# facebookresearch/momentum

Hardware: NVIDIA H100
Metric: GN iterations/sec (batched 72-joint IK) (higher is better)
Workload: dtype f32

## Files before the change

momentum_b200/csrc/ik_capi.cu:

```cuda
#include "../../include/momentum_b200.h"

#include <cuda_runtime.h>
#include <nvtx3/nvToolsExt.h>

#include <algorithm>
#include <cfloat>
#include <cmath>
#include <cstdio>
#include <cstdlib>
#include <cstring>
#include <memory>
#include <string>
#include <vector>

#include "ik_chol_sched.h"
#include "ik_fused.cuh"
#include "ik_jtj_tc.cuh"
#include "ik_kernels.cuh"
#include "ik_plan.h"
#include "ik_solve_path.h"

using namespace mb2;

namespace {
// ... 139 lines not shown
  DeviceBuffer<ContribDesc> dContribs;
  DeviceBuffer<float> dLimitData;
  DeviceBuffer<int32_t> dEnabledList, dIdentity, dDeviceCols;
  DeviceBuffer<float> dTargets, dWeights, dJ, dTheta, dState, dH, dTargetStage;
  DeviceBuffer<double> dErrors;
  DeviceBuffer<double> dJacobi;
  std::unique_ptr<DeviceSchedule> sched;
  SweepLaunch lastSweep[2]{};
  FunctionTables tables() const;
};

struct PhaseEvent {
  cudaEvent_t start, stop;
  int phase;
};

struct mb2_solver {
  mb2_solver_function* fn{nullptr};
  mb2_gauss_newton_options opt{};
  DeviceBuffer<float> dH, dDelta, dThetaOrig, dTheta0, dScale, dGradDotDelta, dThetaStage, dGrad, dTiles, dRadius, dRSaved;
  DeviceBuffer<double> dLastErrors, dTrialErrors, dHistory;
  DeviceBuffer<int32_t> dActive, dIterations, dStatus, dSearching, dActiveCount, dWorkCounter, dQrChunks;
  DeviceBuffer<unsigned long long> dPhaseCycles;
  DeviceBuffer<float> dPark;
  DeviceBuffer<uint32_t> dParkSlots;
  SolvePath path;
  cudaEvent_t fusedStart{nullptr}, fusedStop{nullptr};
  double fusedMs{0};
  int* hActiveCount{nullptr};
  char* hResults{nullptr};
  size_t hResultsBytes{0};
  bool resultsStaged{false};
  uint64_t totalIterations{0}, kernelLaunches{0};
  bool profiling{false};
  bool inKernelProfile{false};
  std::vector<PhaseEvent> events;
  double phaseMs[4]{0, 0, 0, 0};
  uint64_t phaseLaunches[4]{0, 0, 0, 0};
  size_t historyStride{0};
  ~mb2_solver() {
    if (hActiveCount) cudaFreeHost(hActiveCount);
    if (hResults) cudaFreeHost(hResults);
    if (fusedStart) cudaEventDestroy(fusedStart);
    if (fusedStop) cudaEventDestroy(fusedStop);
    for (auto& e : events) { cudaEventDestroy(e.start); cudaEventDestroy(e.stop); }
  }
};

// ... 1397 lines not shown
  c.tilesStride = tilesStride;
  TrQrArgs t{};
  t.q.c = c;
  t.q.jacobian = f->dJ.p;
  t.q.numCols = f->plan.numCols;
  t.q.ldJ = f->ldJ;
  t.q.chunkStart = s->dQrChunks.p;
  t.q.numChunks = int32_t(P.qrChunkStarts.size()) - 1;
  t.T = f->tables();
  t.targets = f->dTargets.p;
  t.cweights = f->dWeights.p;
  t.radius = s->dRadius.p;
  t.rSaved = s->dRSaved.p;
  t.maxRadius = 10.f;
  t.maxChunkRows = P.qrWidestChunk;
  GramCholArgs gc{};
  gc.g = g;
  gc.c = c;
  gc.c.tilesIn = nullptr;
  gc.phaseCycles = s->inKernelProfile ? s->dPhaseCycles.p : nullptr;
  GramCholGlobalTables gt{};
  if (P.kind == kSolveGramCholesky) {
    const DeviceSchedule& ds = *f->sched;
    gc.parkTiles = ds.gc.parkTiles;
    if (gc.parkTiles > 0) {
      const int slots = gramCholeskyParkSlots(gc, ds.dev, ds.gcParams != nullptr);
      if (slots < 1) {
        s->path = SolvePath{};
        return fail(MB2_ERR_CUDA, "Gram + Cholesky fusion: no resident CTA");
      }
      if (s->dParkSlots.n < size_t(slots / 32)) {
        MB2_CUDA(s->dParkSlots.resize(size_t(slots / 32)));
        MB2_CUDA(cudaMemsetAsync(s->dParkSlots.p, 0, s->dParkSlots.n * sizeof(uint32_t), st));
      }
      MB2_CUDA(s->dPark.resize(size_t(slots) * size_t(gc.parkTiles) * 256));
      gc.park = s->dPark.p;
      gc.parkSlots = s->dParkSlots.p;
      gc.parkSlotWords = int32_t(slots / 32);
    }
    gt.L = ds.gc.L;
    gt.tab = ds.gcTab.p;
  }
  CholArgs& step = qr ? t.q.c : (P.kind == kSolveGramCholesky ? gc.c : c);
  SweepArgs trial = sweepArgs(f, theta, s->dSearching.p);
  trial.errors = s->dTrialErrors.p;
  LineSearchArgs la{};
  la.batch = B; la.ns = ns; la.numParams = n; la.ldTheta = n;
  la.errors = f->dErrors.p;
  la.trialErrors = s->dTrialErrors.p;
  la.gradDotDelta = s->dGradDotDelta.p;
  la.scale = s->dScale.p;
  la.searching = s->dSearching.p;
  la.subsetVariant = o.subset_line_search;
  la.active = s->dActive.p;
  BookkeepingArgs ba{};
  ba.batch = B;
  ba.errors = f->dErrors.p; ba.lastErrors = s->dLastErrors.p; ba.active = s->dActive.p; ba.iterations = s->dIterations.p;
  ba.status = s->dStatus.p; ba.history = history;
  ba.theta = theta; ba.ldTheta = n; ba.numParams = n;
  ba.minIterations = minIt; ba.maxIterations = maxIt; ba.threshold = o.threshold; ba.activeCount = s->dActiveCount.p;

  s->kernelLaunches = 0;
// ... 235 lines not shown
```

momentum_b200/csrc/ik_chol_sched.cpp:

```cpp
#include "ik_chol_sched.h"

#include "ik_chol_sched.cuh"

#include <algorithm>
#include <cstdio>
#include <cstdlib>
#include <map>
#include <set>
#include <tuple>

namespace mb2 {

namespace {

struct BitRows {
  int n, words;
  std::vector<uint64_t> b;
  BitRows(int n_) : n(n_), words((n_ + 63) / 64), b(size_t(n_) * ((n_ + 63) / 64), 0) {}
  uint64_t* row(int i) { return b.data() + size_t(i) * words; }
  const uint64_t* row(int i) const { return b.data() + size_t(i) * words; }
  void set(int i, int j) { row(i)[j >> 6] |= 1ull << (j & 63); }
  void clear(int i, int j) { row(i)[j >> 6] &= ~(1ull << (j & 63)); }
  bool test(int i, int j) const { return (row(i)[j >> 6] >> (j & 63)) & 1ull; }
  int count(int i) const {
// ... 342 lines not shown
      if (stripsOfQuad[q] != stripsOfQuad[q0] || stripId[{q, K}] != stripId[{q0, K}] + (q - q0) * stripsOfQuad[q0]) return "Gram plan: row quads of one unit are not laid out uniformly";
  }
  out.colStripStart.assign(T + 1, 0);
  for (int K = 0; K < T; ++K) {
    out.colStripStart[K + 1] = out.colStripStart[K] + int(ofCol[K].size());
    out.colStrip.insert(out.colStrip.end(), ofCol[K].begin(), ofCol[K].end());
  }
  return "";
}

void makeGramBlob(const GramPlan& g, const CholSchedule& s, std::vector<int32_t>& blob, int32_t offsets[8]) {
  blob.clear();
  int k = 0;
  auto add = [&](const std::vector<int32_t>& v) { offsets[k++] = int32_t(blob.size()); blob.insert(blob.end(), v.begin(), v.end()); while (blob.size() % 4) blob.push_back(0); };
  add(g.tileOrder); add(g.tileQuadStart); add(g.quad); add(std::vector<int32_t>()); add(g.colStripStart); add(g.colStrip);
  std::vector<int32_t> stripRow(g.numStrips), info(s.numTiles);
  for (int i = 0; i < g.numStrips; ++i) stripRow[i] = g.stripCoord[2 * i];
  auto validOf = [&](int K) { int v = 0; while (v < kCholTile && s.perm[16 * K + v] >= 0) ++v; return v; };
  for (int t = 0; t < s.numTiles; ++t) info[t] = validOf(s.tileRow[t]) | (validOf(s.tileCol[t]) << 8) | ((s.tileRow[t] == s.tileCol[t] ? 1 : 0) << 16);
  add(stripRow); add(info);
  if (blob.empty()) blob.push_back(0);
}

std::string makeGramCholTables(const GramPlan& g, const CholSchedule& s, GramCholTables& out) {
  out = GramCholTables();
  std::vector<uint16_t>& t = out.tab;
  bool fits = true;
  auto put = [&](int64_t v) { fits = fits && v >= 0 && v <= 0xFFFF; t.push_back(uint16_t(v)); };
  auto section = [&]() { while (t.size() % 4) t.push_back(0); return int32_t(t.size()); };
  auto validOf = [&](int K) { int v = 0; while (v < kCholTile && s.perm[16 * K + v] >= 0) ++v; return v; };
  out.L.gram = section();
  for (int32_t tile : g.tileOrder) {
    if (tile < 0) { put(0xFFFF); put(0); put(0); put(0); continue; }
    fits = fits && tile < 0xFFFF;
    put(tile);
    put(validOf(s.tileRow[tile]) | (validOf(s.tileCol[tile]) << 8) | ((s.tileRow[tile] == s.tileCol[tile] ? 1 : 0) << 15));
    put(g.tileQuadStart[tile]); put(g.tileQuadStart[tile + 1]);
  }
  out.L.quad = section();
  for (int32_t v : g.quad) put(v);
  out.L.col = section();
  for (int32_t v : g.colStripStart) put(v);
  out.L.colEnt = section();
  for (int32_t sidx : g.colStrip) { put(int64_t(sidx) * 64); put(g.stripCoord[2 * sidx]); }
  out.L.level = section();
  for (int L = 0; L <= s.numLevels; ++L) { put(s.levelColStart[L]); put(s.levelPanelStart[L]); put(s.levelOrderStart8[L]); put(s.levelVTaskStart[L]); }
  out.L.diag = section();
  for (int32_t K : s.levelCols) { put(K); put(s.diagTile[K]); put(s.colPanelStart[K]); put(s.colPanelStart[K + 1]); }
  out.L.panel = section();
  for (size_t pi = 0; pi < s.panelTile.size(); ++pi) { put(s.panelTile[pi]); put(s.panelDiag[pi]); }
  out.L.order = section();
  for (int32_t ti : s.taskOrder8) {
    if (ti < 0) { put(0xFFFF); put(0); put(0); put(0); continue; }
    fits = fits && s.taskDst[ti] < 0xFFFF;
    put(s.taskDst[ti]); put(s.taskPairStart[ti]); put(s.taskPairStart[ti + 1]); put(0);
  }
  out.L.pair = section();
  for (size_t p = 0; p < s.pairA.size(); ++p) { put(s.pairA[p]); put(s.pairB[p]); }
  out.L.vtask = section();
  for (size_t vi = 0; vi < s.vtaskRow.size(); ++vi) { put(s.vtaskRow[vi]); put(s.vtaskSrcStart[vi]); put(s.vtaskSrcStart[vi + 1]); put(0); }
  out.L.vsrc = section();
  for (size_t p = 0; p < s.vsrcTile.size(); ++p) { put(s.vsrcTile[p]); put(s.vsrcCol[p]); }
  out.L.colPanel = section();
  for (size_t p = 0; p < s.colPanelTile.size(); ++p) { put(s.colPanelTile[p]); put(s.colPanelRow[p]); }
  section();
  const int64_t onStrips = (int64_t(g.stride) + 64 + 255) / 256;
  out.parkTiles = int32_t(std::min<int64_t>(s.numTiles, onStrips));
  return fits ? "" : "Gram + Cholesky tables: an entry does not fit in 16 bits";
}

void layoutDeviceColumns(CholSchedule& s, std::vector<int32_t>& deviceColumnOrder) {
  deviceColumnOrder.clear();
  s.nParams = s.n;
  for (int K = 0; K < s.numTileCols; ++K) {
    while (deviceColumnOrder.size() % 4 != 0) deviceColumnOrder.push_back(-1);
    for (int j = 0; j < kCholTile; ++j) {
      int16_t& p = s.perm[16 * K + j];
      if (p < 0) continue;
      const int dev = int(deviceColumnOrder.size());
      deviceColumnOrder.push_back(p);
      p = int16_t(dev);
    }
  }
  s.n = int32_t(deviceColumnOrder.size());
  s.pos.assign(s.n, int16_t(-1));
  for (int slot = 0; slot < s.nPad; ++slot) if (s.perm[slot] >= 0) s.pos[s.perm[slot]] = int16_t(slot);
  s.order.assign(deviceColumnOrder.begin(), deviceColumnOrder.end());
}

}

// ... 43 lines not shown
```

momentum_b200/csrc/ik_chol_sched.h:

```cpp
#pragma once

#include <cstdint>
#include <string>
#include <vector>

namespace mb2 {

constexpr int kCholTile = 16;

struct CholSchedule {
  int32_t n{0}, nPad{0}, numTileCols{0}, numTiles{0}, numLevels{0};
  int32_t nParams{0};
  std::vector<int16_t> perm;
  std::vector<int16_t> pos;
  std::vector<int16_t> tileIdTable;
  std::vector<int16_t> tileRow, tileCol;
  std::vector<int32_t> diagTile;
  std::vector<int32_t> levelColStart, levelCols;
  std::vector<int32_t> levelPanelStart, panelTile, panelDiag, panelRow;
  std::vector<int32_t> levelTaskStart, taskDst, taskPairStart, pairA, pairB;
  std::vector<int32_t> levelOrderStart8, taskOrder8, levelOrderStart16, taskOrder16;
  std::vector<int32_t> levelVTaskStart, vtaskRow, vtaskSrcStart, vsrcTile, vsrcCol;
  std::vector<int32_t> colPanelStart, colPanelTile, colPanelRow;
  std::vector<int> order;
// ... 12 lines not shown
  std::vector<int32_t> stripCoord;
  std::vector<int32_t> tileOrder;
  std::vector<int32_t> tilePairStart;
  std::vector<int32_t> pairA, pairB;
  std::vector<int32_t> tileQuadStart;
  std::vector<int32_t> quad;
  std::vector<int32_t> colStripStart;
  std::vector<int32_t> colStrip;
  std::vector<uint32_t> cellStripOff;
  std::vector<uint16_t> cellQuadStride;
  int32_t residOff{0};
  int32_t stride{0};
  int64_t macs{0};
};
std::string buildGramPlan(const CholSchedule& s, const std::vector<int32_t>& cellRow0, const std::vector<int32_t>& cellRows, const std::vector<int32_t>& cellCol,
                          int numRows, GramPlan& out);

void makeGramBlob(const GramPlan& g, const CholSchedule& s, std::vector<int32_t>& blob, int32_t offsets[8]);

struct CholSchedDev;
void makeScheduleBlob(const CholSchedule& s, std::vector<int32_t>& blob, CholSchedDev& dev);

struct GramCholLayout {
  int32_t gram, quad, col, colEnt, level, diag, panel, order, pair, vtask, vsrc, colPanel;
};
struct GramCholTables {
  GramCholLayout L{};
  std::vector<uint16_t> tab;
  int32_t parkTiles{0};
};
std::string makeGramCholTables(const GramPlan& g, const CholSchedule& s, GramCholTables& out);

}
```

momentum_b200/csrc/ik_kernels.cu:

```cuda
#include "ik_kernels.cuh"

#include <algorithm>
#include <cstdio>
#include <type_traits>

#include "ik_chol.cuh"
#include "ik_chol_sched.h"
#include "ik_jtj_tc.cuh"
#include "ik_ptx.cuh"
#include "ik_device.cuh"
#include "ik_jacobi.cuh"

namespace mb2 {

__device__ __forceinline__ double warpSum(double v) {
  for (int o = 16; o > 0; o >>= 1) v += __shfl_xor_sync(0xffffffffu, v, o);
  return v;
}

size_t sweepSmemPerInstance(const FunctionTables& T, int warpsPerInstance) {
  const size_t nPad = (T.numParams + 3) & ~3;
  const size_t jp = warpsPerInstance > 1 ? size_t((T.numJoints * kParametersPerJoint + 1) & ~1) : 0;
  return sizeof(float) * (nPad + jp + size_t((T.numJoints * kJointStateStride + 1) & ~1) + size_t((T.recStride + 1) & ~1) + 4 + 2 * size_t(warpsPerInstance));
}
// ... 1874 lines not shown
  const bool prof = (a.profile & 1) != 0;
  cudaError_t e;
  if (wide) e = prof ? cudaFuncSetAttribute(choleskyScheduledKernel<512, true>, cudaFuncAttributeMaxDynamicSharedMemorySize, int(smem))
                     : cudaFuncSetAttribute(choleskyScheduledKernel<512, false>, cudaFuncAttributeMaxDynamicSharedMemorySize, int(smem));
  else e = prof ? cudaFuncSetAttribute(choleskyScheduledKernel<256, true>, cudaFuncAttributeMaxDynamicSharedMemorySize, int(smem))
                : cudaFuncSetAttribute(choleskyScheduledKernel<256, false>, cudaFuncAttributeMaxDynamicSharedMemorySize, int(smem));
  if (e != cudaSuccess) return e;
  if (a.tilesIn == nullptr && (a.g == nullptr || a.ldG != cholGradientLd(a.ns))) return cudaErrorInvalidValue;
  if ((a.ldH & 3) != 0 || (a.hStride & 3) != 0 || (a.tilesStride & 3) != 0) return cudaErrorInvalidValue;
  CUtensorMap hmap;
  const bool fromGram = a.tilesIn != nullptr;
  const uint64_t dims[3] = {uint64_t(fromGram ? 256 : a.ldH), uint64_t(fromGram ? sched.numTiles : a.ns + 1), uint64_t(a.batch)};
  const uint64_t strides[2] = {uint64_t(fromGram ? 256 : a.ldH) * sizeof(float), uint64_t(fromGram ? a.tilesStride : a.hStride) * sizeof(float)};
  const uint32_t box[3] = {16u, 16u, 1u};
  e = makeTensorMap3d(&hmap, fromGram ? a.tilesIn : a.H, dims, strides, box, 64);
  if (e != cudaSuccess) return e;
  if (wide && prof) choleskyScheduledKernel<512, true><<<a.batch, 512, smem, stream>>>(hmap, a, sched);
  else if (wide) choleskyScheduledKernel<512, false><<<a.batch, 512, smem, stream>>>(hmap, a, sched);
  else if (prof) choleskyScheduledKernel<256, true><<<a.batch, 256, smem, stream>>>(hmap, a, sched);
  else choleskyScheduledKernel<256, false><<<a.batch, 256, smem, stream>>>(hmap, a, sched);
  return cudaGetLastError();
}

__device__ int acquireParkSlot(uint32_t* words, int numWords, int start) {
  for (int w = start % numWords;; w = (w + 1 == numWords) ? 0 : w + 1) {
    uint32_t freeBits = ~__ldcg(words + w);
    while (freeBits != 0u) {
      const int bit = __ffs(freeBits) - 1;
      if ((atomicOr(words + w, 1u << bit) & (1u << bit)) == 0u) return 32 * w + bit;
      freeBits &= freeBits - 1u;
    }
  }
}

template <bool kProfile, class Tables>
__global__ void __launch_bounds__(kGramThreads, 4) gramCholeskyKernel(const GramCholArgs a, const CholSchedDev S, const __grid_constant__ Tables P) {
  extern __shared__ __align__(16) float gcSmem[];
  const GramArgs& g = a.g;
  const CholArgs& c = a.c;
  const int b = blockIdx.x;
  if (c.active[b] == 0) return;
  const int n = c.ns, tid = threadIdx.x;
  const int warp = tid >> 5, lane = tid & 31, hw = tid >> 4, hl = tid & 15;
  constexpr int kWarps = kGramThreads / 32;
  float* U = gcSmem + (((128u - (smemAddr(gcSmem) & 127u)) & 127u) >> 2);
  const size_t tileFloats = size_t(S.numTiles) * 256, sweepFloats = g.stripStride + 64;
  const size_t uni = ((tileFloats > sweepFloats ? tileFloats : sweepFloats) + 3) & ~size_t(3);
  float* strips = U;
  float* resid = U + g.residOff;
  float* tiles = U;
  float* y = U + uni;
  float* gsub = y + S.nPad;
  int* flags = reinterpret_cast<int*>(gsub + ((n + 3) & ~3));
  unsigned long long* bar = reinterpret_cast<unsigned long long*>(flags + 4);
  const uint16_t* tab = P.tab;
  const GramCholLayout& L = P.L;
  long long pc[8] = {0, 0, 0, 0, 0, 0, 0, 0}, pt = 0;
  if constexpr (kProfile) pt = clock64();
#define MB2_GC(k) if constexpr (kProfile) { const long long now = clock64(); pc[k] += now - pt; pt = now; }
  const uint32_t barAddr = smemAddr(bar);
  const uint32_t stripBytes = uint32_t(g.stripStride) * 4u;
  if (tid == 0) {
    flags[0] = 0;
    mbarInit(barAddr, 1);
    fenceBarrierInit();
    mbarExpectTx(barAddr, stripBytes);
    const char* src = reinterpret_cast<const char*>(g.strips + size_t(b) * g.stripStride);
    for (uint32_t off = 0; off < stripBytes; off += 16384u) bulkLoad(smemAddr(strips) + off, src + off, stripBytes - off < 16384u ? stripBytes - off : 16384u, barAddr);
    flags[1] = a.parkTiles > 0 ? acquireParkSlot(a.parkSlots, a.parkSlotWords, b) : 0;
  }
  if (tid >= 64 && tid < 128) strips[g.stripStride + (tid - 64)] = 0.f;
  __syncthreads();
  mbarWaitRelaxed(barAddr, 0);
  MB2_GC(0)
  float* park = a.park + size_t(flags[1]) * size_t(a.parkTiles) * 256 + 4 * lane;
  const int rounds = g.numOrder / kWarps;
  auto tileInfoOf = [](int packed) { return (packed & 0x7FFF) | ((packed >> 15) << 16); };
  for (int r = 0; r < rounds; ++r) {
    const int4 rec = tableRecord4(tab + L.gram + 4 * (r * kWarps + warp));
    if (rec.x == 0xFFFF) continue;
    float acc[2][4];
#pragma unroll
    for (int i = 0; i < 2; ++i)
#pragma unroll
      for (int j = 0; j < 4; ++j) acc[i][j] = 0.f;
    gramTileAccumulate(strips, tab + L.quad, rec.z, rec.w, lane, acc);
    if (rec.x >= a.parkTiles) gramTileStore(tiles + size_t(rec.x) * 256, acc, tileInfoOf(rec.y), g.regularization, lane);
    else {
      __stcg(reinterpret_cast<float4*>(park + size_t(rec.x) * 256), make_float4(acc[0][0], acc[0][1], acc[0][2], acc[0][3]));
      __stcg(reinterpret_cast<float4*>(park + size_t(rec.x) * 256 + 128), make_float4(acc[1][0], acc[1][1], acc[1][2], acc[1][3]));
    }
  }
  for (int K = hw; K < S.numTileCols; K += kGramThreads / 16)
    y[16 * K + hl] = gramVectorEntry(strips, resid, tab + L.colEnt, int(tab[L.col + K]), int(tab[L.col + K + 1]), hl);
  __syncthreads();
  MB2_GC(1)
  for (int r = 0; r < rounds; ++r) {
    const int4 rec = tableRecord4(tab + L.gram + 4 * (r * kWarps + warp));
    if (rec.x == 0xFFFF || rec.x >= a.parkTiles) continue;
    const float4 v0 = __ldcg(reinterpret_cast<const float4*>(park + size_t(rec.x) * 256));
    const float4 v1 = __ldcg(reinterpret_cast<const float4*>(park + size_t(rec.x) * 256 + 128));
    const float acc[2][4] = {{v0.x, v0.y, v0.z, v0.w}, {v1.x, v1.y, v1.z, v1.w}};
    gramTileStore(tiles + size_t(rec.x) * 256, acc, tileInfoOf(rec.y), g.regularization, lane);
  }
  for (int s2 = tid; s2 < S.nPad; s2 += kGramThreads) {
    const int p = S.perm[s2];
    if (p >= 0) gsub[p] = y[s2];
  }
  __syncthreads();
  if (tid == 0 && a.parkTiles > 0) atomicAnd(a.parkSlots + (flags[1] >> 5), ~(1u << (flags[1] & 31)));
  MB2_GC(2)
  for (int Lv = 0; Lv < S.numLevels; ++Lv) {
    const int4 l0 = tableRecord4(tab + L.level + 4 * Lv), l1 = tableRecord4(tab + L.level + 4 * (Lv + 1));
    for (int ci = l0.x + warp; ci < l1.x; ci += kWarps) {
      const int4 d = tableRecord4(tab + L.diag + 4 * ci);
      cholDiagTile(tiles + size_t(d.y) * 256, y + 16 * d.x, lane, c.regularization, flags);
    }
    __syncthreads();
    MB2_GC(3)
    for (int pi = l0.y + warp; pi < l1.y; pi += kWarps) {
      const int2 pe = tableRecord2(tab + L.panel + 2 * pi);
      float* ptile = tiles + size_t(pe.x) * 256;
      float x[2][4];
      cholPanelProduct(ptile, tiles + size_t(pe.y) * 256, lane, x);
      cholPanelStore(ptile, lane, x);
    }
    __syncthreads();
    MB2_GC(4)
    for (int oi = l0.z + warp; oi < l1.z; oi += kWarps) {
      const int4 o = tableRecord4(tab + L.order + 4 * oi);
      if (o.x != 0xFFFF) cholUpdateTile(tiles, tab + L.pair, tab + L.pair + 1, 2, o.y, o.z, o.x, lane);
    }
    for (int vi = l0.w + hw; vi < l1.w; vi += kGramThreads / 16) {
// ... 8 lines not shown
    for (int ci = c0 + warp; ci < c1; ci += kWarps) {
      const int4 d = tableRecord4(tab + L.diag + 4 * ci);
      cholBackwardPanels(tiles, y, tab + L.colPanel, tab + L.colPanel + 1, 2, d.z, d.w, d.x, d.y, lane);
    }
    __syncthreads();
  }
  MB2_GC(6)
  cholFinish(c, b, n, y, gsub, flags[0] != 0, S.pos);
  MB2_GC(7)
  if constexpr (kProfile) {
    if (b == int(gridDim.x >> 1) && tid == 0 && a.phaseCycles != nullptr)
      for (int k = 0; k < 8; ++k) a.phaseCycles[k] += (unsigned long long)pc[k];
  }
#undef MB2_GC
}

template <bool kProfile, class Tables>
static cudaError_t prepareGramCholesky(size_t smem) {
  cudaError_t e = cudaFuncSetAttribute(gramCholeskyKernel<kProfile, Tables>, cudaFuncAttributeMaxDynamicSharedMemorySize, int(smem));
  if (e != cudaSuccess) return e;
  return cudaFuncSetAttribute(gramCholeskyKernel<kProfile, Tables>, cudaFuncAttributePreferredSharedMemoryCarveout, int(cudaSharedmemCarveoutMaxShared));
}

int gramCholeskyParkSlots(const GramCholArgs& a, const CholSchedDev& sched, bool paramTables) {
  const size_t smem = gramCholeskySmemBytes(a.g.stripStride, a.c.ns, sched.nPad, sched.numTiles);
  cudaError_t e = paramTables ? prepareGramCholesky<false, GramCholParamTables>(smem) : prepareGramCholesky<false, GramCholGlobalTables>(smem);
  int perSm = 0;
  if (e == cudaSuccess)
    e = paramTables ? cudaOccupancyMaxActiveBlocksPerMultiprocessor(&perSm, gramCholeskyKernel<false, GramCholParamTables>, kGramThreads, smem)
                    : cudaOccupancyMaxActiveBlocksPerMultiprocessor(&perSm, gramCholeskyKernel<false, GramCholGlobalTables>, kGramThreads, smem);
  if (e != cudaSuccess || perSm < 1) return -1;
  return (g_numSms * perSm + 31) / 32 * 32;
}

cudaError_t launchGramCholesky(const GramCholArgs& a, const CholSchedDev& sched, const GramCholParamTables* inParams, const GramCholGlobalTables& inGlobal, bool profile,
                               cudaStream_t stream) {
  const size_t smem = gramCholeskySmemBytes(a.g.stripStride, a.c.ns, sched.nPad, sched.numTiles);
  if (smem > size_t(g_maxSmemOptin) || (a.g.stripStride & 3) != 0) return cudaErrorInvalidConfiguration;
  if (a.parkTiles > 0 && (a.park == nullptr || a.parkSlots == nullptr || a.parkSlotWords < 1)) return cudaErrorInvalidValue;
  cudaError_t e;
  if (inParams != nullptr) e = profile ? prepareGramCholesky<true, GramCholParamTables>(smem) : prepareGramCholesky<false, GramCholParamTables>(smem);
  else e = profile ? prepareGramCholesky<true, GramCholGlobalTables>(smem) : prepareGramCholesky<false, GramCholGlobalTables>(smem);
  if (e != cudaSuccess) return e;
  if (inParams != nullptr) {
    if (profile) gramCholeskyKernel<true, GramCholParamTables><<<a.c.batch, kGramThreads, smem, stream>>>(a, sched, *inParams);
    else gramCholeskyKernel<false, GramCholParamTables><<<a.c.batch, kGramThreads, smem, stream>>>(a, sched, *inParams);
  } else {
    if (profile) gramCholeskyKernel<true, GramCholGlobalTables><<<a.c.batch, kGramThreads, smem, stream>>>(a, sched, inGlobal);
    else gramCholeskyKernel<false, GramCholGlobalTables><<<a.c.batch, kGramThreads, smem, stream>>>(a, sched, inGlobal);
  }
  return cudaGetLastError();
}

}
#include "ik_qr.cuh"
#include "ik_tr_qr.cuh"
namespace mb2 {

cudaError_t initKernelAttributes() {
  int dev = 0;
  cudaError_t e = cudaGetDevice(&dev);
  if (e != cudaSuccess) return e;
// ... 99 lines not shown
```

momentum_b200/csrc/ik_kernels.cuh:

```cuda
#pragma once

#include <cuda_runtime.h>

#include "ik_chol_sched.cuh"
#include "ik_chol_sched.h"
#include "ik_solve_path.h"
#include "ik_types.h"

namespace mb2 {

struct SweepArgs {
  FunctionTables T;
  int32_t batch;
  const float* theta;
  int32_t ldTheta;
  const float* targets;
  const float* cweights;
  float* jacobian;
  double* errors;
  const int32_t* active;
  float* stateOut;
  int32_t stageTables;
  int32_t warpsPerInstance;
};
// ... 41 lines not shown
};

struct GramArgs {
  int32_t batch;
  const float* strips;
  size_t stripStride;
  int32_t residOff;
  const int32_t* active;
  int32_t numStrips, numTiles, numTileCols, nPad;
  int32_t numOrder;
  const int32_t* blob;
  int32_t blobInts;
  int32_t offTileOrder, offTilePairStart, offPairA, offPairB, offColStripStart, offColStrip, offStripRow, offTileInfo;
  float regularization;
  float* out;
  size_t outStride;
};
cudaError_t launchGramTiles(const GramArgs& a, int threads, cudaStream_t stream);

struct GramCholArgs {
  GramArgs g;
  CholArgs c;
  unsigned long long* phaseCycles;
  float* park;
  uint32_t* parkSlots;
  int32_t parkSlotWords, parkTiles;
};
constexpr int kGramCholParamEntries = 8192;
struct alignas(16) GramCholParamTables {
  GramCholLayout L;
  uint16_t tab[kGramCholParamEntries];
};
struct GramCholGlobalTables {
  GramCholLayout L;
  const uint16_t* tab;
};
int gramCholeskyParkSlots(const GramCholArgs& a, const CholSchedDev& sched, bool paramTables);
cudaError_t launchGramCholesky(const GramCholArgs& a, const CholSchedDev& sched, const GramCholParamTables* inParams, const GramCholGlobalTables& inGlobal, bool profile,
                               cudaStream_t stream);

struct QrArgs {
  CholArgs c;
  const float* jacobian;
  int32_t numCols, ldJ;
  const int32_t* chunkStart;
  int32_t numChunks;
};
struct TrQrArgs {
  QrArgs q;
  FunctionTables T;
  const float* targets;
  const float* cweights;
  float* radius;
  float* rSaved;
  float maxRadius;
  int32_t maxChunkRows;
};
cudaError_t launchTrustRegionQr(const TrQrArgs& a, cudaStream_t stream);
cudaError_t launchQrSolve(const QrArgs& a, int maxChunkRows, cudaStream_t stream);
struct SkeletonStateArgs {
// ... 165 lines not shown
```

momentum_b200/csrc/ik_solve_path.cpp:

```cpp
#include "ik_solve_path.h"

#include <algorithm>
#include <cstring>

#include "ik_chol.cuh"

namespace mb2 {

std::vector<int32_t> makeFusedBlob(const HostCharacter& h, const Plan& p, const std::vector<int32_t>& gramBlob, const std::vector<int32_t>& schedBlob, FusedBlobLayout& L) {
  std::vector<int32_t> blob;
  auto add = [&](const void* data, size_t bytes) {
    const int32_t off = int32_t(blob.size());
    const size_t words = (bytes + 3) / 4;
    blob.resize(blob.size() + words, 0);
    if (bytes) std::memcpy(blob.data() + off, data, bytes);
    while (blob.size() % 4) blob.push_back(0);
    return off;
  };
  L.parent = add(h.parent.data(), h.parent.size() * 4);
  L.offset = add(h.offset.data(), h.offset.size() * 4);
  L.prerot = add(h.prerot.data(), h.prerot.size() * 4);
  L.ptOuter = add(h.ptOuter.data(), h.ptOuter.size() * 4);
  L.ptInner = add(h.ptInner.data(), h.ptInner.size() * 4);
  L.ptVals = add(h.ptVals.data(), h.ptVals.size() * 4);
// ... 10 lines not shown
  L.sched = add(schedBlob.data(), schedBlob.size() * 4);
  if (blob.empty()) blob.push_back(0);
  while (blob.size() % 4) blob.push_back(0);
  L.words = int32_t(blob.size());
  return blob;
}

size_t cholSmemBytes(int n, int NB, bool matrixInSmem) {
  const size_t ldp = ((n + 1 + 3) & ~3) + 4;
  size_t s = sizeof(float) * (NB * ldp + ((n + 3) & ~3)) + 4 * sizeof(int);
  if (matrixInSmem) s += sizeof(float) * size_t(n + 1) * (n | 1);
  return s;
}

size_t gramTilesSmemBytes(size_t stripStride, int blobInts) { return 128 + sizeof(float) * (stripStride + 64) + 16 + sizeof(int32_t) * size_t((blobInts + 3) & ~3); }

size_t choleskyScheduledSmemBytes(int n, int nPad, int numTiles, int blobInts) {
  return 1024  + sizeof(float) * (size_t(numTiles) * 256 + size_t(nPad) + 2 * size_t((n + 3) & ~3)) +
         sizeof(int32_t) * size_t((blobInts + 3) & ~3) + 32;
}

size_t gramCholeskySmemBytes(size_t stripStride, int n, int nPad, int numTiles) {
  const size_t uni = std::max<size_t>(size_t(numTiles) * 256, stripStride + 64);
  return 128 + sizeof(float) * (((uni + 3) & ~size_t(3)) + size_t(nPad) + size_t((n + 3) & ~3)) + 32;
}

size_t qrSmemFloats(int n, int maxChunkRows) {
  return (size_t(n) * (n + 1) / 2 + 3 & ~size_t(3)) + 3 * size_t((n + 3) & ~3) + size_t((n + 4) & ~3) + size_t(n + 1) * size_t(maxChunkRows | 1) + 8;
}
int qrMaxChunkRows(int n, size_t smemBytes) {
  const size_t fixed = qrSmemFloats(n, 0) - size_t(n + 1);
  const size_t floats = smemBytes / sizeof(float);
  if (floats <= fixed + size_t(n + 1) * 9) return 0;
  int p = int((floats - fixed) / size_t(n + 1)) - 1;
  p = std::min(p, 128) & ~1;
  return p;
}

size_t trQrSmemFloats(int n, int numParams, int numJoints, int maxChunkRows) {
  const size_t packed = (size_t(n) * (n + 1) / 2 + 3) & ~size_t(3);
  const size_t n4 = size_t((n + 3) & ~3), np4 = size_t((numParams + 3) & ~3);
  const size_t chunk = (size_t(n + 1) * size_t(maxChunkRows | 1) + 3) & ~size_t(3);
  return packed + std::max(packed, chunk) + 7 * n4 + size_t((n + 4) & ~3) + 2 * np4 + size_t((numJoints * kJointStateStride + 3) & ~3) + 64;
}

bool jtjTensorShape(int ns, int numCols, int ldJ) { return ns >= 1 && ns <= numCols && numCols + 1 <= 512 && (ldJ % kJtjKBlock) == 0; }

// ... 60 lines not shown
    useSchedule = false;
    useGram = false;
    if ((rc = request(1, false, false)) != MB2_OK) return rc;
  }
  const int ns = F.numCols;
  if (ns <= 0) return refuse(MB2_ERR_INVALID_ARGUMENT, "no enabled parameters");
  if (useGram && gramTilesSmemBytes(size_t(F.stripStride), F.gramBlobInts) > size_t(200 * 1024)) {
    if (o.jtj_mode == MB2_JTJ_SPARSE_TILES) return refuse(MB2_ERR_UNSUPPORTED, "Jacobian strips do not fit in shared memory for this system");
    useGram = false;
    if ((rc = request(2, cholMode == 2, false)) != MB2_OK) return rc;
  }
  const bool eligible = useGram && useSchedule && o.do_line_search == 0 && P.fused.groups >= 1;
  if (o.fused_mode == MB2_FUSED_PERSISTENT && !eligible)
    return refuse(MB2_ERR_UNSUPPORTED, "the fused kernel needs the tile-sparse Gram + tile-scheduled Cholesky path, no line search, and a plan that fits in shared memory");
  if (eligible && (o.fused_mode == MB2_FUSED_PERSISTENT || (o.fused_mode == MB2_FUSED_AUTO && batch <= P.fused.groups * lim.numSms))) {
    P.kind = kSolvePersistent;
    P.jtjMode = MB2_JTJ_SPARSE_TILES;
    return MB2_OK;
  }
  bool useGramChol = false;
  if (useGram && useSchedule) {
    const int rounds = std::max(F.orderEntries / kGramWarps, 1);
    const bool fits = gramCholeskySmemBytes(size_t(F.stripStride), ns, F.nPad, F.numTiles) <= size_t(200 * 1024) && rounds <= kGramCholMaxRounds && F.gramCholValid;
    if (o.fused_mode == MB2_FUSED_GRAM_CHOLESKY && !fits) return refuse(MB2_ERR_UNSUPPORTED, "Gram + Cholesky fusion: strips / tiles of this plan do not fit in shared memory, or too many tiles per warp");
    useGramChol = fits && (o.fused_mode == MB2_FUSED_AUTO || o.fused_mode == MB2_FUSED_GRAM_CHOLESKY);
  } else if (o.fused_mode == MB2_FUSED_GRAM_CHOLESKY) {
    return refuse(MB2_ERR_UNSUPPORTED, "Gram + Cholesky fusion needs the tile-sparse Gram + tile-scheduled Cholesky path");
  }
  P.jtjMode = useGram ? MB2_JTJ_SPARSE_TILES : resolveJtjMode(o.jtj_mode == MB2_JTJ_SPARSE_TILES ? MB2_JTJ_AUTO : o.jtj_mode, F.jtjTensor);
  if (P.jtjMode < 0) return refuse(MB2_ERR_UNSUPPORTED, "tensor-core JtJ does not support this shape");
  if (useQr) {
    int rows = qrMaxChunkRows(ns, size_t(200 * 1024));
    if (rows < 8) return refuse(MB2_ERR_UNSUPPORTED, "the QR step keeps R in shared memory: too many enabled parameters for this kernel");
    if (useTr) {
      rows = std::min(rows, std::max(8, ns / 2));
      if (trQrSmemFloats(ns, ch.numParams, ch.numJoints, rows) * sizeof(float) > size_t(220 * 1024))
        return refuse(MB2_ERR_UNSUPPORTED, "the trust-region QR kernel keeps R and the damping rows in shared memory: too many enabled parameters / joints");
      P.trRSavedFloats = (size_t(ns) * (ns + 1) / 2 + 3) & ~size_t(3);
    }
    P.qrMaxChunkRows = rows;
    P.qrChunkStarts.assign(1, 0);
    int r0 = 0, widest = 0;
    for (const auto& ef : fn.efs) {
      if (!(ef.weight > 0.f)) continue;
      const int size = jacobianBlockSize(ch, ef);
      for (int done = 0; done < size; done += rows) { const int p = std::min(rows, size - done); P.qrChunkStarts.push_back(r0 + done + p); widest = std::max(widest, p); }
      r0 += size;
// ... 27 lines not shown
```

Measured before the change: 9.653 million.

## Replace global park buffer with slot placement and mbarrier region waits in Gram+Cholesky

After: 9.635 million (median of 6 runs). No clear change (-0.2%).

```diff
diff --git a/momentum_b200/csrc/ik_capi.cu b/momentum_b200/csrc/ik_capi.cu
--- a/momentum_b200/csrc/ik_capi.cu
+++ b/momentum_b200/csrc/ik_capi.cu
@@ -185,8 +185,6 @@
   DeviceBuffer<double> dLastErrors, dTrialErrors, dHistory;
   DeviceBuffer<int32_t> dActive, dIterations, dStatus, dSearching, dActiveCount, dWorkCounter, dQrChunks;
   DeviceBuffer<unsigned long long> dPhaseCycles;
-  DeviceBuffer<float> dPark;
-  DeviceBuffer<uint32_t> dParkSlots;
   SolvePath path;
   cudaEvent_t fusedStart{nullptr}, fusedStop{nullptr};
   double fusedMs{0};
@@ -1630,22 +1628,6 @@
   GramCholGlobalTables gt{};
   if (P.kind == kSolveGramCholesky) {
     const DeviceSchedule& ds = *f->sched;
-    gc.parkTiles = ds.gc.parkTiles;
-    if (gc.parkTiles > 0) {
-      const int slots = gramCholeskyParkSlots(gc, ds.dev, ds.gcParams != nullptr);
-      if (slots < 1) {
-        s->path = SolvePath{};
-        return fail(MB2_ERR_CUDA, "Gram + Cholesky fusion: no resident CTA");
-      }
-      if (s->dParkSlots.n < size_t(slots / 32)) {
-        MB2_CUDA(s->dParkSlots.resize(size_t(slots / 32)));
-        MB2_CUDA(cudaMemsetAsync(s->dParkSlots.p, 0, s->dParkSlots.n * sizeof(uint32_t), st));
-      }
-      MB2_CUDA(s->dPark.resize(size_t(slots) * size_t(gc.parkTiles) * 256));
-      gc.park = s->dPark.p;
-      gc.parkSlots = s->dParkSlots.p;
-      gc.parkSlotWords = int32_t(slots / 32);
-    }
     gt.L = ds.gc.L;
     gt.tab = ds.gcTab.p;
   }
diff --git a/momentum_b200/csrc/ik_chol_sched.cpp b/momentum_b200/csrc/ik_chol_sched.cpp
--- a/momentum_b200/csrc/ik_chol_sched.cpp
+++ b/momentum_b200/csrc/ik_chol_sched.cpp
@@ -388,8 +388,56 @@
   if (blob.empty()) blob.push_back(0);
 }
 
+namespace {
+
+std::string placeGramTiles(const GramPlan& g, const std::vector<int32_t>& quads, int numTiles, std::vector<int32_t>& slot, std::vector<int32_t>& wait, int& onStrips) {
+  const int rounds = int(g.tileOrder.size()) / kGramWarps;
+  onStrips = int(std::min<int64_t>(numTiles, (int64_t(g.stride) + 64 + 255) / 256));
+  std::vector<int> need(numTiles, -1), roundOf(numTiles, -1);
+  for (int s = 0; s < onStrips; ++s) need[s] = 0;
+  for (int r = 0; r < rounds; ++r)
+    for (int w = 0; w < kGramWarps; ++w) {
+      const int t = g.tileOrder[size_t(r) * kGramWarps + w];
+      if (t < 0) continue;
+      if (t >= numTiles || roundOf[t] >= 0) return "Gram plan: the tile order does not hold every tile once";
+      roundOf[t] = r;
+      for (int q = g.tileQuadStart[t]; q < g.tileQuadStart[t + 1]; ++q)
+        for (int k = 0; k < 4; ++k) {
+          const int s = quads[4 * size_t(q) + k] / 256;
+          if (s < onStrips) need[s] = std::max(need[s], r + 1);
+        }
+    }
+  for (int t = 0; t < numTiles; ++t)
+    if (roundOf[t] < 0) return "Gram plan: the tile order does not hold every tile once";
+  std::vector<int> slots(numTiles), tiles(numTiles);
+  for (int i = 0; i < numTiles; ++i) slots[i] = tiles[i] = i;
+  std::stable_sort(slots.begin(), slots.end(), [&](int a, int b) { return need[a] > need[b]; });
+  std::stable_sort(tiles.begin(), tiles.end(), [&](int a, int b) { return roundOf[a] > roundOf[b]; });
+  slot.assign(numTiles, -1);
+  wait.assign(numTiles, -1);
+  for (int i = 0; i < numTiles; ++i) {
+    const int t = tiles[i], s = slots[i];
+    if (need[s] > roundOf[t] + 1) return "Gram + Cholesky tables: no tile placement over the dead strips";
+    slot[t] = s;
+    wait[t] = need[s];
+  }
+  return "";
+}
+
+}
+
 std::string makeGramCholTables(const GramPlan& g, const CholSchedule& s, GramCholTables& out) {
   out = GramCholTables();
+  const int64_t uni = (std::max<int64_t>(int64_t(s.numTiles) * 256, int64_t(g.stride) + 64) + 3) & ~int64_t(3);
+  out.L.zeroStrip = ((s.n + 3) & ~3) >= 64 ? int32_t(uni + s.nPad) : g.stride;
+  std::vector<int32_t> quads(g.quad);
+  for (int32_t& o : quads) if (o == g.stride) o = out.L.zeroStrip;
+  std::vector<int32_t> wait;
+  const std::string placed = placeGramTiles(g, quads, s.numTiles, out.slot, wait, out.slotsOnStrips);
+  if (!placed.empty()) return placed;
+  out.rounds = int32_t(g.tileOrder.size()) / kGramWarps;
+  if (out.rounds + 1 > 31) return "Gram + Cholesky tables: more region barriers than the record holds";
+  const std::vector<int32_t>& sl = out.slot;
   std::vector<uint16_t>& t = out.tab;
   bool fits = true;
   auto put = [&](int64_t v) { fits = fits && v >= 0 && v <= 0xFFFF; t.push_back(uint16_t(v)); };
@@ -398,13 +446,13 @@
   out.L.gram = section();
   for (int32_t tile : g.tileOrder) {
     if (tile < 0) { put(0xFFFF); put(0); put(0); put(0); continue; }
-    fits = fits && tile < 0xFFFF;
-    put(tile);
-    put(validOf(s.tileRow[tile]) | (validOf(s.tileCol[tile]) << 8) | ((s.tileRow[tile] == s.tileCol[tile] ? 1 : 0) << 15));
+    fits = fits && sl[tile] < 0xFFFF;
+    put(sl[tile]);
+    put(validOf(s.tileRow[tile]) | (validOf(s.tileCol[tile]) << 5) | ((s.tileRow[tile] == s.tileCol[tile] ? 1 : 0) << 10) | ((wait[tile] + 1) << 11));
     put(g.tileQuadStart[tile]); put(g.tileQuadStart[tile + 1]);
   }
   out.L.quad = section();
-  for (int32_t v : g.quad) put(v);
+  for (int32_t v : quads) put(v);
   out.L.col = section();
   for (int32_t v : g.colStripStart) put(v);
   out.L.colEnt = section();
@@ -412,27 +460,83 @@
   out.L.level = section();
   for (int L = 0; L <= s.numLevels; ++L) { put(s.levelColStart[L]); put(s.levelPanelStart[L]); put(s.levelOrderStart8[L]); put(s.levelVTaskStart[L]); }
   out.L.diag = section();
-  for (int32_t K : s.levelCols) { put(K); put(s.diagTile[K]); put(s.colPanelStart[K]); put(s.colPanelStart[K + 1]); }
+  for (int32_t K : s.levelCols) { put(K); put(sl[s.diagTile[K]]); put(s.colPanelStart[K]); put(s.colPanelStart[K + 1]); }
   out.L.panel = section();
-  for (size_t pi = 0; pi < s.panelTile.size(); ++pi) { put(s.panelTile[pi]); put(s.panelDiag[pi]); }
+  for (size_t pi = 0; pi < s.panelTile.size(); ++pi) { put(sl[s.panelTile[pi]]); put(sl[s.panelDiag[pi]]); }
   out.L.order = section();
   for (int32_t ti : s.taskOrder8) {
     if (ti < 0) { put(0xFFFF); put(0); put(0); put(0); continue; }
-    fits = fits && s.taskDst[ti] < 0xFFFF;
-    put(s.taskDst[ti]); put(s.taskPairStart[ti]); put(s.taskPairStart[ti + 1]); put(0);
+    fits = fits && sl[s.taskDst[ti]] < 0xFFFF;
+    put(sl[s.taskDst[ti]]); put(s.taskPairStart[ti]); put(s.taskPairStart[ti + 1]); put(0);
   }
   out.L.pair = section();
-  for (size_t p = 0; p < s.pairA.size(); ++p) { put(s.pairA[p]); put(s.pairB[p]); }
+  for (size_t p = 0; p < s.pairA.size(); ++p) { put(sl[s.pairA[p]]); put(sl[s.pairB[p]]); }
   out.L.vtask = section();
   for (size_t vi = 0; vi < s.vtaskRow.size(); ++vi) { put(s.vtaskRow[vi]); put(s.vtaskSrcStart[vi]); put(s.vtaskSrcStart[vi + 1]); put(0); }
   out.L.vsrc = section();
-  for (size_t p = 0; p < s.vsrcTile.size(); ++p) { put(s.vsrcTile[p]); put(s.vsrcCol[p]); }
+  for (size_t p = 0; p < s.vsrcTile.size(); ++p) { put(sl[s.vsrcTile[p]]); put(s.vsrcCol[p]); }
   out.L.colPanel = section();
-  for (size_t p = 0; p < s.colPanelTile.size(); ++p) { put(s.colPanelTile[p]); put(s.colPanelRow[p]); }
+  for (size_t p = 0; p < s.colPanelTile.size(); ++p) { put(sl[s.colPanelTile[p]]); put(s.colPanelRow[p]); }
+  out.L.perm = section();
+  for (int16_t p : s.perm) put(p < 0 ? 0xFFFF : p);
+  fits = fits && s.nPad < 0xFFFF && out.L.zeroStrip + 64 <= 0xFFFF;
   section();
-  const int64_t onStrips = (int64_t(g.stride) + 64 + 255) / 256;
-  out.parkTiles = int32_t(std::min<int64_t>(s.numTiles, onStrips));
-  return fits ? "" : "Gram + Cholesky tables: an entry does not fit in 16 bits";
+  if (!fits) return "Gram + Cholesky tables: an entry does not fit in 16 bits";
+  if (getenv("MB2_SCHED_DUMP") != nullptr) {
+    std::vector<int> perBarrier(out.rounds + 2, 0);
+    for (int tile = 0; tile < s.numTiles; ++tile) ++perBarrier[wait[tile] + 1];
+    fprintf(stderr, "gram + cholesky storage: %d tiles, %d rounds, %d slots on the strips; stored at once %d, after barrier j:", s.numTiles, out.rounds, out.slotsOnStrips, perBarrier[0]);
+    for (int j = 0; j <= out.rounds; ++j) fprintf(stderr, " %d", perBarrier[j + 1]);
+    fprintf(stderr, "\n");
+  }
+  return checkGramCholStorage(out, s.numTiles, g.stride);
+}
+
+std::string checkGramCholStorage(const GramCholTables& t, int numTiles, int stride) {
+  const int rounds = t.rounds, barriers = rounds + 1;
+  const int onStrips = int(std::min<int64_t>(numTiles, (int64_t(stride) + 64 + 255) / 256));
+  std::vector<int> owner(numTiles, -1);
+  std::vector<int> lastRead(numTiles, -1);
+  for (int r = 0; r < rounds; ++r)
+    for (int w = 0; w < kGramWarps; ++w) {
+      const uint16_t* rec = t.tab.data() + t.L.gram + 4 * (r * kGramWarps + w);
+      if (rec[0] == 0xFFFF) continue;
+      if (rec[0] >= numTiles) return "storage check: a slot outside the union buffer";
+      if (owner[rec[0]] >= 0) return "storage check: two tiles share a slot";
+      owner[rec[0]] = r;
+      for (int q = rec[2]; q < rec[3]; ++q)
+        for (int k = 0; k < 4; ++k) {
+          const int s = t.tab[t.L.quad + 4 * q + k] / 256;
+          if (s < numTiles) lastRead[s] = std::max(lastRead[s], r);
+        }
+    }
+  for (int s = 0; s < numTiles; ++s)
+    if (owner[s] < 0) return "storage check: a slot holds no tile";
+  for (int r = 0; r < rounds; ++r)
+    for (int w = 0; w < kGramWarps; ++w) {
+      const uint16_t* rec = t.tab.data() + t.L.gram + 4 * (r * kGramWarps + w);
+      if (rec[0] == 0xFFFF) continue;
+      const int wait = (rec[1] >> 11) - 1;
+      if (wait >= barriers) return "storage check: a wait on a barrier that does not exist";
+      if (rec[0] < onStrips && (wait < 0 || wait < lastRead[rec[0]] + 1)) return "storage check: a tile can be written over a strip that is still read";
+    }
+  std::vector<int> arrived(barriers, 0), pc(kGramWarps, 0), inWait(kGramWarps, 0);
+  for (int w = 0; w < kGramWarps; ++w) ++arrived[0];
+  for (bool moved = true; moved;) {
+    moved = false;
+    for (int w = 0; w < kGramWarps; ++w)
+      while (pc[w] < rounds) {
+        const uint16_t* rec = t.tab.data() + t.L.gram + 4 * (pc[w] * kGramWarps + w);
+        if (!inWait[w]) { ++arrived[pc[w] + 1]; inWait[w] = 1; moved = true; }
+        const int wait = rec[0] == 0xFFFF ? -1 : (rec[1] >> 11) - 1;
+        if (wait >= 0 && arrived[wait] < kGramWarps) break;
+        inWait[w] = 0;
+        ++pc[w];
+      }
+  }
+  for (int w = 0; w < kGramWarps; ++w)
+    if (pc[w] < rounds) return "storage check: the region waits deadlock";
+  return "";
 }
 
 void layoutDeviceColumns(CholSchedule& s, std::vector<int32_t>& deviceColumnOrder) {
diff --git a/momentum_b200/csrc/ik_chol_sched.h b/momentum_b200/csrc/ik_chol_sched.h
--- a/momentum_b200/csrc/ik_chol_sched.h
+++ b/momentum_b200/csrc/ik_chol_sched.h
@@ -58,13 +58,16 @@
 void makeScheduleBlob(const CholSchedule& s, std::vector<int32_t>& blob, CholSchedDev& dev);
 
 struct GramCholLayout {
-  int32_t gram, quad, col, colEnt, level, diag, panel, order, pair, vtask, vsrc, colPanel;
+  int32_t gram, quad, col, colEnt, level, diag, panel, order, pair, vtask, vsrc, colPanel, perm;
+  int32_t zeroStrip;
 };
 struct GramCholTables {
   GramCholLayout L{};
   std::vector<uint16_t> tab;
-  int32_t parkTiles{0};
+  std::vector<int32_t> slot;
+  int32_t rounds{0};
+  int32_t slotsOnStrips{0};
 };
 std::string makeGramCholTables(const GramPlan& g, const CholSchedule& s, GramCholTables& out);
-
+std::string checkGramCholStorage(const GramCholTables& t, int numTiles, int stride);
 }
diff --git a/momentum_b200/csrc/ik_kernels.cu b/momentum_b200/csrc/ik_kernels.cu
--- a/momentum_b200/csrc/ik_kernels.cu
+++ b/momentum_b200/csrc/ik_kernels.cu
@@ -1920,17 +1920,6 @@
   return cudaGetLastError();
 }
 
-__device__ int acquireParkSlot(uint32_t* words, int numWords, int start) {
-  for (int w = start % numWords;; w = (w + 1 == numWords) ? 0 : w + 1) {
-    uint32_t freeBits = ~__ldcg(words + w);
-    while (freeBits != 0u) {
-      const int bit = __ffs(freeBits) - 1;
-      if ((atomicOr(words + w, 1u << bit) & (1u << bit)) == 0u) return 32 * w + bit;
-      freeBits &= freeBits - 1u;
-    }
-  }
-}
-
 template <bool kProfile, class Tables>
 __global__ void __launch_bounds__(kGramThreads, 4) gramCholeskyKernel(const GramCholArgs a, const CholSchedDev S, const __grid_constant__ Tables P) {
   extern __shared__ __align__(16) float gcSmem[];
@@ -1956,57 +1945,47 @@
   long long pc[8] = {0, 0, 0, 0, 0, 0, 0, 0}, pt = 0;
   if constexpr (kProfile) pt = clock64();
 #define MB2_GC(k) if constexpr (kProfile) { const long long now = clock64(); pc[k] += now - pt; pt = now; }
-  const uint32_t barAddr = smemAddr(bar);
+  const uint32_t barAddr = smemAddr(bar), regionAddr = barAddr + 8u;
   const uint32_t stripBytes = uint32_t(g.stripStride) * 4u;
+  const int rounds = g.numOrder / kWarps;
   if (tid == 0) {
     flags[0] = 0;
     mbarInit(barAddr, 1);
+    for (int j = 0; j <= rounds; ++j) mbarInit(regionAddr + 8u * uint32_t(j), kWarps);
     fenceBarrierInit();
     mbarExpectTx(barAddr, stripBytes);
     const char* src = reinterpret_cast<const char*>(g.strips + size_t(b) * g.stripStride);
     for (uint32_t off = 0; off < stripBytes; off += 16384u) bulkLoad(smemAddr(strips) + off, src + off, stripBytes - off < 16384u ? stripBytes - off : 16384u, barAddr);
-    flags[1] = a.parkTiles > 0 ? acquireParkSlot(a.parkSlots, a.parkSlotWords, b) : 0;
-  }
-  if (tid >= 64 && tid < 128) strips[g.stripStride + (tid - 64)] = 0.f;
+  }
+  if (tid >= 64 && tid < 128) U[L.zeroStrip + (tid - 64)] = 0.f;
   __syncthreads();
   mbarWaitRelaxed(barAddr, 0);
   MB2_GC(0)
-  float* park = a.park + size_t(flags[1]) * size_t(a.parkTiles) * 256 + 4 * lane;
-  const int rounds = g.numOrder / kWarps;
-  auto tileInfoOf = [](int packed) { return (packed & 0x7FFF) | ((packed >> 15) << 16); };
+  auto tileInfoOf = [](int packed) { return (packed & 31) | (((packed >> 5) & 31) << 8) | (((packed >> 10) & 1) << 16); };
+  for (int K = hw; K < S.numTileCols; K += kGramThreads / 16)
+    y[16 * K + hl] = gramVectorEntry(strips, resid, tab + L.colEnt, int(tab[L.col + K]), int(tab[L.col + K + 1]), hl);
+  __syncwarp();
+  if (lane == 0) mbarArrive(regionAddr);
   for (int r = 0; r < rounds; ++r) {
     const int4 rec = tableRecord4(tab + L.gram + 4 * (r * kWarps + warp));
+    float acc[2][4];
+#pragma unroll
+    for (int i = 0; i < 2; ++i)
+#pragma unroll
+      for (int j = 0; j < 4; ++j) acc[i][j] = 0.f;
+    if (rec.x != 0xFFFF) gramTileAccumulate(strips, tab + L.quad, rec.z, rec.w, lane, acc);
+    __syncwarp();
+    if (lane == 0) mbarArrive(regionAddr + 8u * uint32_t(r + 1));
     if (rec.x == 0xFFFF) continue;
-    float acc[2][4];
-#pragma unroll
-    for (int i = 0; i < 2; ++i)
-#pragma unroll
-      for (int j = 0; j < 4; ++j) acc[i][j] = 0.f;
-    gramTileAccumulate(strips, tab + L.quad, rec.z, rec.w, lane, acc);
-    if (rec.x >= a.parkTiles) gramTileStore(tiles + size_t(rec.x) * 256, acc, tileInfoOf(rec.y), g.regularization, lane);
-    else {
-      __stcg(reinterpret_cast<float4*>(park + size_t(rec.x) * 256), make_float4(acc[0][0], acc[0][1], acc[0][2], acc[0][3]));
-      __stcg(reinterpret_cast<float4*>(park + size_t(rec.x) * 256 + 128), make_float4(acc[1][0], acc[1][1], acc[1][2], acc[1][3]));
-    }
-  }
-  for (int K = hw; K < S.numTileCols; K += kGramThreads / 16)
-    y[16 * K + hl] = gramVectorEntry(strips, resid, tab + L.colEnt, int(tab[L.col + K]), int(tab[L.col + K + 1]), hl);
+    if ((rec.y >> 11) != 0) mbarWaitSilent<false>(regionAddr + 8u * uint32_t((rec.y >> 11) - 1), 0);
+    gramTileStore(tiles + size_t(rec.x) * 256, acc, tileInfoOf(rec.y), g.regularization, lane);
+  }
+  MB2_GC(1)
   __syncthreads();
-  MB2_GC(1)
-  for (int r = 0; r < rounds; ++r) {
-    const int4 rec = tableRecord4(tab + L.gram + 4 * (r * kWarps + warp));
-    if (rec.x == 0xFFFF || rec.x >= a.parkTiles) continue;
-    const float4 v0 = __ldcg(reinterpret_cast<const float4*>(park + size_t(rec.x) * 256));
-    const float4 v1 = __ldcg(reinterpret_cast<const float4*>(park + size_t(rec.x) * 256 + 128));
-    const float acc[2][4] = {{v0.x, v0.y, v0.z, v0.w}, {v1.x, v1.y, v1.z, v1.w}};
-    gramTileStore(tiles + size_t(rec.x) * 256, acc, tileInfoOf(rec.y), g.regularization, lane);
-  }
   for (int s2 = tid; s2 < S.nPad; s2 += kGramThreads) {
-    const int p = S.perm[s2];
-    if (p >= 0) gsub[p] = y[s2];
-  }
-  __syncthreads();
-  if (tid == 0 && a.parkTiles > 0) atomicAnd(a.parkSlots + (flags[1] >> 5), ~(1u << (flags[1] & 31)));
+    const int p = tab[L.perm + s2];
+    if (p != 0xFFFF) gsub[p] = y[s2];
+  }
   MB2_GC(2)
   for (int Lv = 0; Lv < S.numLevels; ++Lv) {
     const int4 l0 = tableRecord4(tab + L.level + 4 * Lv), l1 = tableRecord4(tab + L.level + 4 * (Lv + 1));
@@ -2061,22 +2040,11 @@
   return cudaFuncSetAttribute(gramCholeskyKernel<kProfile, Tables>, cudaFuncAttributePreferredSharedMemoryCarveout, int(cudaSharedmemCarveoutMaxShared));
 }
 
-int gramCholeskyParkSlots(const GramCholArgs& a, const CholSchedDev& sched, bool paramTables) {
-  const size_t smem = gramCholeskySmemBytes(a.g.stripStride, a.c.ns, sched.nPad, sched.numTiles);
-  cudaError_t e = paramTables ? prepareGramCholesky<false, GramCholParamTables>(smem) : prepareGramCholesky<false, GramCholGlobalTables>(smem);
-  int perSm = 0;
-  if (e == cudaSuccess)
-    e = paramTables ? cudaOccupancyMaxActiveBlocksPerMultiprocessor(&perSm, gramCholeskyKernel<false, GramCholParamTables>, kGramThreads, smem)
-                    : cudaOccupancyMaxActiveBlocksPerMultiprocessor(&perSm, gramCholeskyKernel<false, GramCholGlobalTables>, kGramThreads, smem);
-  if (e != cudaSuccess || perSm < 1) return -1;
-  return (g_numSms * perSm + 31) / 32 * 32;
-}
-
 cudaError_t launchGramCholesky(const GramCholArgs& a, const CholSchedDev& sched, const GramCholParamTables* inParams, const GramCholGlobalTables& inGlobal, bool profile,
                                cudaStream_t stream) {
   const size_t smem = gramCholeskySmemBytes(a.g.stripStride, a.c.ns, sched.nPad, sched.numTiles);
   if (smem > size_t(g_maxSmemOptin) || (a.g.stripStride & 3) != 0) return cudaErrorInvalidConfiguration;
-  if (a.parkTiles > 0 && (a.park == nullptr || a.parkSlots == nullptr || a.parkSlotWords < 1)) return cudaErrorInvalidValue;
+  if (a.g.numOrder % kGramWarps != 0 || a.g.numOrder / kGramWarps > kGramCholMaxRounds) return cudaErrorInvalidValue;
   cudaError_t e;
   if (inParams != nullptr) e = profile ? prepareGramCholesky<true, GramCholParamTables>(smem) : prepareGramCholesky<false, GramCholParamTables>(smem);
   else e = profile ? prepareGramCholesky<true, GramCholGlobalTables>(smem) : prepareGramCholesky<false, GramCholGlobalTables>(smem);
diff --git a/momentum_b200/csrc/ik_kernels.cuh b/momentum_b200/csrc/ik_kernels.cuh
--- a/momentum_b200/csrc/ik_kernels.cuh
+++ b/momentum_b200/csrc/ik_kernels.cuh
@@ -87,9 +87,6 @@
   GramArgs g;
   CholArgs c;
   unsigned long long* phaseCycles;
-  float* park;
-  uint32_t* parkSlots;
-  int32_t parkSlotWords, parkTiles;
 };
 constexpr int kGramCholParamEntries = 8192;
 struct alignas(16) GramCholParamTables {
@@ -100,7 +97,6 @@
   GramCholLayout L;
   const uint16_t* tab;
 };
-int gramCholeskyParkSlots(const GramCholArgs& a, const CholSchedDev& sched, bool paramTables);
 cudaError_t launchGramCholesky(const GramCholArgs& a, const CholSchedDev& sched, const GramCholParamTables* inParams, const GramCholGlobalTables& inGlobal, bool profile,
                                cudaStream_t stream);
 
diff --git a/momentum_b200/csrc/ik_solve_path.cpp b/momentum_b200/csrc/ik_solve_path.cpp
--- a/momentum_b200/csrc/ik_solve_path.cpp
+++ b/momentum_b200/csrc/ik_solve_path.cpp
@@ -56,7 +56,7 @@
 
 size_t gramCholeskySmemBytes(size_t stripStride, int n, int nPad, int numTiles) {
   const size_t uni = std::max<size_t>(size_t(numTiles) * 256, stripStride + 64);
-  return 128 + sizeof(float) * (((uni + 3) & ~size_t(3)) + size_t(nPad) + size_t((n + 3) & ~3)) + 32;
+  return 128 + sizeof(float) * (((uni + 3) & ~size_t(3)) + size_t(nPad) + size_t((n + 3) & ~3)) + 16 + 8 * (2 + kGramCholMaxRounds);
 }
 
 size_t qrSmemFloats(int n, int maxChunkRows) {
@@ -163,7 +163,8 @@
   if (useGram && useSchedule) {
     const int rounds = std::max(F.orderEntries / kGramWarps, 1);
     const bool fits = gramCholeskySmemBytes(size_t(F.stripStride), ns, F.nPad, F.numTiles) <= size_t(200 * 1024) && rounds <= kGramCholMaxRounds && F.gramCholValid;
-    if (o.fused_mode == MB2_FUSED_GRAM_CHOLESKY && !fits) return refuse(MB2_ERR_UNSUPPORTED, "Gram + Cholesky fusion: strips / tiles of this plan do not fit in shared memory, or too many tiles per warp");
+    if (o.fused_mode == MB2_FUSED_GRAM_CHOLESKY && !fits)
+      return refuse(MB2_ERR_UNSUPPORTED, "Gram + Cholesky fusion: strips / tiles of this plan do not fit in shared memory, or too many tiles per warp, or no tile placement over the dead strips");
     useGramChol = fits && (o.fused_mode == MB2_FUSED_AUTO || o.fused_mode == MB2_FUSED_GRAM_CHOLESKY);
   } else if (o.fused_mode == MB2_FUSED_GRAM_CHOLESKY) {
     return refuse(MB2_ERR_UNSUPPORTED, "Gram + Cholesky fusion needs the tile-sparse Gram + tile-scheduled Cholesky path");
```
